# importZL/semantic_segmentation

Hardware: AMD Instinct MI355X
Metric: images/sec (fwd+bwd) U-Net 256x256 bs=32 per GPU (higher is better)
Workload: dtype f16; 1 GPU; unet.UNet(1,2) 256x256 fwd+bwd, CE+Dice loss, batch 32/GPU (BASELINE configs[1]); global_batch=32, parallelism=dp1, dice=per-rank

## Files before the change

### include/gsseg.h

```cpp
#ifndef GSSEG_H
#define GSSEG_H

#include <stdint.h>

#ifdef __cplusplus
extern "C" {
#endif

#define GS_ABI_VERSION 52

enum GsDtype { GS_F16 = 0, GS_BF16 = 1 };
enum GsStatus { GS_OK = 0, GS_EINVAL = -1, GS_ELAUNCH = -2, GS_EUNSUPPORTED = -3 };
enum GsAct { GS_ACT_NONE = 0, GS_ACT_RELU = 1, GS_ACT_LEAKY02 = 2, GS_ACT_TANH = 3 };

#define GS_MAX_TAPS 64

typedef struct GsConvGeom {
    int32_t N, IH, IW, Cin, in_pix_stride, in_coff;
    int32_t OHg, OWg, Cout;
    int32_t OH, OW, out_pix_stride, out_coff;
    int32_t isy, isx, osy, osx, ooy, oox;
    int32_t ntaps;
    int32_t tap_dy[GS_MAX_TAPS], tap_dx[GS_MAX_TAPS];
    int32_t tap_w[GS_MAX_TAPS];
// ... 85 lines not shown
                    int dtype, void* stream);

int gs_bn_bwd_tiles(int N, int H, int W);
int gs_bn_bwd_tiles_used(int N, int H, int W, int pooled);
int gs_bn_act_bwd_reduce(const void* y, const void* dz_a, int sa, int coff_a, const void* dzp,
                         const void* dz_b, int act_b, const uint8_t* keep_mask, float keep_scale,
                         const float* scale, const float* shift, const float* mean, const float* invstd, int act,
                         float* partials, int N, int H, int W, int C, int dtype, void* stream);
int gs_bn_bwd_coeffs(const float* partials, int ntiles, int C, double count, float gscale, float* dgamma,
                     float* dbeta, float* c1, float* c2, void* stream);
int gs_bn_act_bwd_apply(const void* y, const void* dz_a, int sa, int coff_a, const void* dzp,
                        const void* dz_b, int act_b, const uint8_t* keep_mask, float keep_scale,
                        const float* scale, const float* shift, const float* mean, const float* invstd,
                        const float* c1, const float* c2, int act, int bn, void* dy, int N, int H, int W, int C,
                        int dtype, void* stream);

int gs_maxpool3d_fwd(const void* z, int z_pix_stride, int z_coff, void* zp, int NB, int D, int H, int W, int C,
                     int dtype, void* stream);
int gs_maxpool3d_fwd_pair(const void* z_hi, const void* z_lo, int z_pix_stride, void* zp_hi, void* zp_lo, int zp_pix_stride,
                          int NB, int D, int H, int W, int C, int dtype, void* stream);
int gs_maxpool3d_fwd_pair_q8(const void* z_hi, const void* z_lo, int z_q8, int zq_coff, int z_pix_stride, void* zp_hi, void* zp_lo,
                             int zp_q8, int zp_pix_stride, int NB, int D, int H, int W, int C, int dtype, void* stream);
int gs_maxpool3d_bwd(const void* z, int z_pix_stride, int z_coff, const void* dzp, const void* dres,
                     int res_pix_stride, int res_coff, void* dz, int NB, int D, int H, int W, int C, int dtype,
                     void* stream);

int gs_maxpool2x2_fwd(const void* z, int z_pix_stride, int z_coff, void* zp, int N, int H, int W, int C, int dtype,
                      void* stream);
int gs_maxpool2x2_fwd_pair(const void* z_hi, const void* z_lo, int z_pix_stride, void* zp_hi, void* zp_lo, int zp_pix_stride, int N, int H,
                           int W, int C, int dtype, void* stream);
// ... 145 lines not shown
int gs_head1x1_bn_fwd_split(const void* y_hi, const void* y_lo, const float* scale, const float* shift, int act, const float* w,
                            const float* bias, float* logits, int N, int H, int W, int Cin, int Cout, int dtype, void* stream);
int gs_stem_fwd_bn_pair(const float* x, const float* w, const float* bn_scale, const float* bn_shift, int act, void* z_hi,
                        void* z_lo, int z_pix_stride, int N, int H, int W, int dtype, void* stream);
int gs_stem_bwd_onepass_strided(const float* x, const void* z, int z_pix_stride, const void* dz, int dz_stride, int dz_coff,
                                int act, float* s1_partials, float* ws, int N, int H, int W, int dtype, void* stream);

int gs_upconv2x2_wgrad_parts(int N, int IH, int IW, int Cin, int Cout);
int64_t gs_upconv2x2_wgrad_ws_floats(int N, int IH, int IW, int Cin, int Cout);
int gs_upconv2x2_wgrad_slabs(const void* x, const void* dy, float* ws, int N, int IH, int IW, int Cin, int x_pix_stride,
                             int x_coff, int Cout, int OH, int OW, int dy_pix_stride, int dy_coff, int ooy, int oox, int dtype,
                             void* stream);

int64_t gs_conv3x3_wgrad_ws_floats(int N, int H, int W, int Cin, int Cout);
int gs_conv3x3_wgrad_parts(int N, int H, int W, int Cin, int Cout);
int gs_conv3x3_wgrad_slabs(const void* x, const void* dy, float* ws, int N, int H, int W, int Cin, int in_pix_stride,
                           int in_coff, int Cout, int out_pix_stride, int out_coff, int dtype, void* stream);
int gs_wgrad_reduce_unpack(const float* ws, int nparts, float* grad, int A, int B, int taps, int transposed,
                           float gscale, void* stream);

int gs_conv3d_3x3x3_mtiles(int NB, int D, int H, int W, int Cout);
int gs_conv3d_3x3x3(const void* x, const void* w, void* y, const float* bias, float* bn_partials, int NB, int D, int H,
                    int W, int Cin, int in_pix_stride, int in_coff, int Cout, int out_pix_stride, int out_coff,
                    const int32_t* tap_dz, const int32_t* tap_dy, const int32_t* tap_dx, int act, int dtype, void* stream);
int gs_conv3d_3x3x3_wgrad(const void* x, const void* dy, float* dw, int NB, int D, int H, int W, int Cin,
                          int in_pix_stride, int in_coff, int Cout, int out_pix_stride, int out_coff, int dtype,
                          void* stream);
int64_t gs_conv3d_3x3x3_wgrad_ws_floats(int NB, int D, int H, int W, int Cin, int Cout);
int gs_conv3d_3x3x3_wgrad_parts(int NB, int D, int H, int W, int Cin, int Cout);
int gs_conv3d_3x3x3_wgrad_slabs(const void* x, const void* dy, float* ws, int NB, int D, int H, int W, int Cin,
// ... 29 lines not shown
```

### semantic_segmentation_amd/_lib.py

```python
from __future__ import annotations

import ctypes
import os
import subprocess
from ctypes import POINTER, c_char_p, c_double, c_float, c_int, c_int32, c_int64, c_void_p

_HERE = os.path.dirname(os.path.abspath(__file__))
LIB_PATH = os.environ.get("GSSEG_LIB", os.path.join(_HERE, "libgsseg_hip.so"))
CSRC = os.path.join(_HERE, "csrc")

GS_F16, GS_BF16 = 0, 1
ACT_NONE, ACT_RELU, ACT_LEAKY02, ACT_TANH = 0, 1, 2, 3
GS_MAX_TAPS = 64
ABI_VERSION = 52


class GsConvGeom(ctypes.Structure):
    _fields_ = [(n, c_int32) for n in (
        "N", "IH", "IW", "Cin", "in_pix_stride", "in_coff", "OHg", "OWg", "Cout", "OH", "OW",
        "out_pix_stride", "out_coff", "isy", "isx", "osy", "osx", "ooy", "oox", "ntaps")] + [
        ("tap_dy", c_int32 * GS_MAX_TAPS), ("tap_dx", c_int32 * GS_MAX_TAPS), ("tap_w", c_int32 * GS_MAX_TAPS)] + [
        (n, c_int32) for n in ("Dg", "Din", "Dout", "isz", "osz", "ooz")] + [("tap_dz", c_int32 * GS_MAX_TAPS)]


class GsPackDesc(ctypes.Structure):
    _fields_ = [("w", c_void_p), ("w_fwd", c_void_p), ("w_dgrad", c_void_p)] + [
        (n, c_int32) for n in ("Cout", "Cin", "taps", "transposed")]


# ... 32 lines not shown
    "gs_conv3d_3x3x3": (c_int, [_P, _P, _P, _F, _F] + [c_int] * 10 + [POINTER(c_int32)] * 3 + [c_int, c_int, c_void_p]),
    "gs_conv3d_3x3x3_wgrad_ws_floats": (c_int64, [c_int] * 6),
    "gs_conv3d_3x3x3_wgrad_parts": (c_int, [c_int] * 6),
    "gs_conv3d_3x3x3_wgrad_slabs": (c_int, [_P, _P, _F] + [c_int] * 11 + [c_void_p]),
    "gs_conv3d_3x3x3_wgrad": (c_int, [_P, _P, _F] + [c_int] * 11 + [c_void_p]),
    "gs_upsample2x_bilinear_fwd": (c_int, [_P, _P] + [c_int] * 13 + [c_void_p]),
    "gs_upsample2x_bilinear_bwd": (c_int, [_P, _P] + [c_int] * 13 + [c_void_p]),
    "gs_affine_warp": (c_int, [_F, _F, _F, c_int, c_int, c_int, c_int, c_float, c_void_p]),
    "gs_optim_chunk_elems": (c_int, []),
    "gs_optim_rmsprop": (c_int, [_P] * 7 + [c_int] + [c_float] * 6 + [c_void_p]),
    "gs_optim_adam": (c_int, [_P] * 7 + [c_int, _P] + [c_float] * 5 + [c_void_p]),
    "gs_conv3x3": (c_int, [_P, _P, _P, _F, _F] + [c_int] * 9 + [POINTER(c_int32), POINTER(c_int32), c_int, c_int, c_void_p]),
    "gs_conv3x3_wgrad": (c_int, [_P, _P, _F] + [c_int] * 10 + [c_void_p]),
    "gs_conv3x3_wgrad_ws_floats": (c_int64, [c_int] * 5),
    "gs_conv3x3_wgrad_parts": (c_int, [c_int] * 5),
    "gs_conv3x3_wgrad_slabs": (c_int, [_P, _P, _F] + [c_int] * 10 + [c_void_p]),
    "gs_wgrad_reduce_unpack": (c_int, [_F, c_int, _F, c_int, c_int, c_int, c_int, c_float, c_void_p]),
    "gs_conv_wgrad": (c_int, [POINTER(GsConvGeom), _P, _P, _F, c_int, c_void_p]),
    "gs_conv_wgrad_assign": (c_int, [POINTER(GsConvGeom), _P, _P, _F, c_int, c_void_p]),
    "gs_conv_wgrad_single_pass": (c_int, [POINTER(GsConvGeom)]),
    "gs_conv_wgrad_parts": (c_int, [POINTER(GsConvGeom)]),
    "gs_conv_wgrad_ws_floats": (c_int64, [POINTER(GsConvGeom)]),
    "gs_conv_wgrad_slabs": (c_int, [POINTER(GsConvGeom), _P, _P, _F, c_int, c_void_p]),
    "gs_conv_wgrad_slabs_batch": (c_int, [c_int, POINTER(POINTER(GsConvGeom)), _P, _P, _F, c_int, c_void_p]),
    "gs_conv_smallcin_mtiles": (c_int, [c_int, c_int, c_int]),
    "gs_conv_smallcin_fwd": (c_int, [_F, _F, _F, _P, _F] + [c_int] * 12 + [c_void_p]),
    "gs_conv_direct_wgrad_ws_floats": (c_int64, [c_int] * 6),
    "gs_conv_smallcin_wgrad": (c_int, [_F, _P, _F, _F] + [c_int] * 10 + [c_float, c_int, c_void_p]),
    "gs_conv_smallcin_dgrad": (c_int, [_P, _F, _F] + [c_int] * 10 + [c_float, c_int, c_void_p]),
    "gs_conv_smallcout_fwd": (c_int, [_P, _F, _F, _F] + [c_int] * 11 + [c_void_p]),
    "gs_conv_smallcout_bwd": (c_int, [_P, _F, _F, _P, _F, _F, _F] + [c_int] * 10 + [c_float, c_int, c_void_p]),
    "gs_bn_partials_floats": (c_int64, [c_int, c_int]),
    "gs_bn_finalize": (c_int, [_F, c_int, c_int, c_double, _F, _F, _F, _F, c_float, c_float, _F, _F, _F, _F, c_void_p]),
    "gs_bn_eval_coeffs": (c_int, [c_int, _F, _F, _F, _F, c_float, _F, _F, _F, _F, c_void_p]),
    "gs_bn_act_apply": (c_int, [_P, _F, _F, c_int, _P, c_int, c_int, _P, _P, c_float] + [c_int] * 5 + [c_void_p]),
    "gs_bn_bwd_tiles": (c_int, [c_int, c_int, c_int]),
    "gs_bn_bwd_tiles_used": (c_int, [c_int, c_int, c_int, c_int]),
    "gs_bn_act_bwd_reduce": (c_int, [_P, _P, c_int, c_int, _P, _P, c_int, _P, c_float, _F, _F, _F, _F, c_int, _F]
                             + [c_int] * 5 + [c_void_p]),
    "gs_bn_bwd_coeffs": (c_int, [_F, c_int, c_int, c_double, c_float, _F, _F, _F, _F, c_void_p]),
    "gs_bn_act_bwd_apply": (c_int, [_P, _P, c_int, c_int, _P, _P, c_int, _P, c_float, _F, _F, _F, _F, _F, _F, c_int,
                                    c_int, _P]
                            + [c_int] * 5 + [c_void_p]),
    "gs_maxpool3d_fwd": (c_int, [_P, c_int, c_int, _P] + [c_int] * 6 + [c_void_p]),
    "gs_maxpool2x2_fwd": (c_int, [_P, c_int, c_int, _P] + [c_int] * 5 + [c_void_p]),
    "gs_maxpool2x2_fwd_pair": (c_int, [_P, _P, c_int, _P, _P, c_int] + [c_int] * 5 + [c_void_p]),
    "gs_maxpool3d_bwd": (c_int, [_P, c_int, c_int, _P, _P, c_int, c_int, _P] + [c_int] * 6 + [c_void_p]),
    "gs_colsum": (c_int, [_P, c_int, c_int] + [c_int] * 8 + [c_float, _F, _F, c_int, c_void_p]),
    "gs_stem_bn_bwd_wgrad": (c_int, [_P, _P, c_int, c_int, _F, _F, _F, _F, _F, _F, _F, c_int, _F, _F, c_int, c_int, c_int,
                                     c_float, c_int, c_void_p]),
    "gs_stem_stats": (c_int, [_F, _F, _F, _F, c_int, c_int, c_int, c_void_p]),
    "gs_stem_bwd_onepass": (c_int, [_F, _P, _P, c_int, c_int, c_int, _F, _F, c_int, c_int, c_int, c_int, c_void_p]),
    "gs_stem_bwd_finalize": (c_int, [_F, _F, _F, _F, _F, _F, _F, c_int, c_float, _F, _F, _F, c_int, c_int, c_int, c_void_p]),
    "gs_stem_fwd_bn": (c_int, [_F, _F, _F, _F, c_int, _P, c_int, c_int, c_int, c_int, c_void_p]),
# ... 118 lines not shown
```

### semantic_segmentation_amd/csrc/bn.hip

```cpp
#include <stdlib.h>

#include "common.hpp"

namespace {

constexpr int RED_SLICES = 64;

__global__ __launch_bounds__(256) void reduce_partials_stage1(const float* __restrict__ part, int ntiles, int C,
                                                              int tiles_per_slice, double* __restrict__ out1) {
    __shared__ double red[2][8][32];
    const int cl = threadIdx.x & 31, tl = threadIdx.x >> 5;
    const int c = blockIdx.x * 32 + cl;
    const int t0 = blockIdx.y * tiles_per_slice, t1 = min(ntiles, t0 + tiles_per_slice);
    double s1 = 0.0, s2 = 0.0;
    if (c < C) {
        for (int tt = t0 + tl; tt < t1; tt += 8) {
            s1 += (double)part[((int64_t)tt * 2 + 0) * C + c];
            s2 += (double)part[((int64_t)tt * 2 + 1) * C + c];
        }
    }
    red[0][tl][cl] = s1;
    red[1][tl][cl] = s2;
    __syncthreads();
    if (tl == 0 && c < C) {
// ... 63 lines not shown
}

template <typename T>
__global__ __launch_bounds__(256) void bn_bwd_coeffs_kernel(const T* __restrict__ s, int nslices, int C, double count,
                                                            float gscale, float* dgamma, float* dbeta, float* c1, float* c2) {
    double s1, s2;
    sum_slices_32x8(s, nslices, C, s1, s2);
    const int c = blockIdx.x * 32 + (threadIdx.x & 31);
    if (c >= C || threadIdx.x >= 32) return;
    if (dbeta) dbeta[c] = (float)(s1 * gscale);
    if (dgamma) dgamma[c] = (float)(s2 * gscale);
    c1[c] = (float)(s1 / count);
    c2[c] = (float)(s2 / count);
}

static int bn_traversal() {
    static const int v = getenv("GSSEG_BN_REV") ? atoi(getenv("GSSEG_BN_REV")) : 3;
    return v;
}

struct ApplyArgs {
    const unsigned short* y;
    const float* scale;
    const float* shift;
    unsigned short* z;
    unsigned short* zp;
    const uint8_t* keep;
    float keep_scale;
    int act, N, H, W, C, zs, zc;
    int rev;
};

template <int DT, bool POOL, bool GENERIC>
// ... 77 lines not shown
    const unsigned short* dzb;
    const uint8_t* keep;
    float keep_scale;
    int act_b;
    const float *scale, *shift, *mean, *invstd, *c1, *c2;
    float* partials;
    unsigned short* dy;
    int sa, ca, act, bn, N, H, W, C;
    int tile_units;
    int rev;
    const float* head_dl;
    const float* head_w;
    int head_n;
};

template <int DT, bool POOL, bool APPLY, bool GENERIC, int HEAD = 0, bool EXTRA = true, bool RN = false>
__global__ __launch_bounds__(256) void bn_act_bwd_kernel(const BwdArgs a) {
    static_assert(!HEAD || (!POOL && !GENERIC), "the head source: plain pixels, slope-family activation");
    static_assert(!(RN && GENERIC), "the rounded slope product belongs to the slope family");
    auto mul_g = [&](float g, float d) __attribute__((always_inline)) { return RN ? mul_rn(g, d) : g * d; };
    constexpr int NH = HEAD ? HEAD : 1;
    constexpr int HEAD_CHUNK = 2048;
    __shared__ float hdl[HEAD ? NH * HEAD_CHUNK : 1];
    __shared__ float red[2][256 * 8 / 8][8];
    const float slope_a = a.act == GS_ACT_RELU ? 0.f : (a.act == GS_ACT_LEAKY02 ? 0.2f : 1.f);
    const float slope_b = a.act_b == GS_ACT_RELU ? 0.f : (a.act_b == GS_ACT_LEAKY02 ? 0.2f : 1.f);
    auto grad_a = [&](float v) __attribute__((always_inline)) { return GENERIC ? act_grad(v, a.act) : (v > 0.f ? 1.f : slope_a); };
    auto grad_b = [&](float v) __attribute__((always_inline)) { return GENERIC ? act_grad(v, a.act_b) : (v > 0.f ? 1.f : slope_b); };
    auto fwd_a = [&](float v) __attribute__((always_inline)) { return GENERIC ? act_fwd(v, a.act) : (v > 0.f ? v : v * slope_a); };
    const int nch = a.C >> 3;
    const int PH = POOL ? (a.H + 1) / 2 : a.H, PW = POOL ? (a.W + 1) / 2 : a.W;
    const int units = a.N * PH * PW;
    const int lanes_per_unit = nch < 256 ? nch : 256;
    const int unit_lanes = 256 / lanes_per_unit;
    const int chl = threadIdx.x % lanes_per_unit, ul = threadIdx.x / lanes_per_unit;
    const int tile = a.rev ? (int)(gridDim.x - 1 - blockIdx.x) : (int)blockIdx.x;
    const int u0 = tile * a.tile_units;
    int u1 = u0 + a.tile_units < units ? u0 + a.tile_units : units;
    if (ul >= unit_lanes) u1 = u0;
    constexpr int UNR = 4;

    for (int ch = chl; ch - chl < nch; ch += lanes_per_unit) {
        const bool ch_ok = ch < nch;
        const int c0 = ch_ok ? ch * 8 : 0;
        if (!ch_ok) u1 = u0;
        float sc[8], sh[8], mu[8], is[8], k1[8], k2[8];
#pragma unroll
        for (int i = 0; i < 8; ++i) {
            sc[i] = a.scale ? a.scale[c0 + i] : 1.f;
            sh[i] = a.shift ? a.shift[c0 + i] : 0.f;
            mu[i] = a.mean ? a.mean[c0 + i] : 0.f;
            is[i] = a.invstd ? a.invstd[c0 + i] : 1.f;
            k1[i] = (APPLY && a.c1) ? a.c1[c0 + i] : 0.f;
            k2[i] = (APPLY && a.c2) ? a.c2[c0 + i] : 0.f;
        }
// ... 361 lines not shown
    GS_CHECK_LAUNCH("gs_bn_act_apply");
    return GS_OK;
}

static int bwd_tile_units(int64_t units) {
    int64_t tu = cdiv64(units, 1024);
    if (tu < 64) tu = 64;
    return (int)tu;
}

extern "C" int gs_bn_bwd_tiles(int N, int H, int W) {
    const int64_t units = (int64_t)N * H * W;
    return (int)cdiv64(units, bwd_tile_units(units));
}

static int launch_bwd(const BwdArgs& a0, bool apply, int dtype, hipStream_t s, int* ntiles_out) {
    BwdArgs a = a0;
    a.rev = (bn_traversal() >> (apply ? 2 : 1)) & 1;
    const bool pool = a.dzp != nullptr;
    const int PH = pool ? (a.H + 1) / 2 : a.H, PW = pool ? (a.W + 1) / 2 : a.W;
    const int64_t units = (int64_t)a.N * PH * PW;
    const int ntiles_max = gs_bn_bwd_tiles(a.N, a.H, a.W);
    a.tile_units = (int)cdiv64(units, ntiles_max);
    if (a.tile_units < 1) a.tile_units = 1;
    const int ntiles = (int)cdiv64(units, a.tile_units);
    if (ntiles_out) *ntiles_out = ntiles;
    const bool generic = a.act == GS_ACT_TANH || (a.dzb && a.act_b == GS_ACT_TANH);
    const bool leaky = !generic && (a.act == GS_ACT_LEAKY02 || (a.dzb && a.act_b == GS_ACT_LEAKY02));
#define LAUNCH(DT, G, R)                                                                                \
    do {                                                                                                \
        if (pool) {                                                                                     \
            if (apply) bn_act_bwd_kernel<DT, true, true, G, 0, true, R><<<ntiles, 256, 0, s>>>(a);      \
            else bn_act_bwd_kernel<DT, true, false, G, 0, true, R><<<ntiles, 256, 0, s>>>(a);           \
        } else if (a.dzb != nullptr || a.keep != nullptr) {                                             \
            if (apply) bn_act_bwd_kernel<DT, false, true, G, 0, true, R><<<ntiles, 256, 0, s>>>(a);     \
            else bn_act_bwd_kernel<DT, false, false, G, 0, true, R><<<ntiles, 256, 0, s>>>(a);          \
        } else {                                                                                        \
            if (apply) bn_act_bwd_kernel<DT, false, true, G, 0, false, R><<<ntiles, 256, 0, s>>>(a);    \
            else bn_act_bwd_kernel<DT, false, false, G, 0, false, R><<<ntiles, 256, 0, s>>>(a);         \
        }                                                                                               \
    } while (0)
    if (a.head_dl != nullptr) {
#define LAUNCH_HEAD(DT, NC, R)                                                                          \
    do {                                                                                                \
        if (apply) bn_act_bwd_kernel<DT, false, true, false, NC, false, R><<<ntiles, 256, 0, s>>>(a);   \
        else bn_act_bwd_kernel<DT, false, false, false, NC, false, R><<<ntiles, 256, 0, s>>>(a);        \
    } while (0)
#define LAUNCH_HEAD_N(DT, R) do { if (a.head_n <= 2) LAUNCH_HEAD(DT, 2, R); else LAUNCH_HEAD(DT, 4, R); } while (0)
        if (dtype == GS_F16) { if (leaky) LAUNCH_HEAD_N(GS_F16, true); else LAUNCH_HEAD_N(GS_F16, false); }
        else { if (leaky) LAUNCH_HEAD_N(GS_BF16, true); else LAUNCH_HEAD_N(GS_BF16, false); }
#undef LAUNCH_HEAD_N
// ... 158 lines not shown
```

### semantic_segmentation_amd/csrc/wgrad3x3.hip

```cpp
#include <stdlib.h>

#include "common.hpp"

namespace {

struct W3Args {
    const unsigned short* x;
    const unsigned short* dy;
    float* dw;
    int N, H, W, Cin, in_stride, in_coff, Cout, out_stride, out_coff;
    int tiles_x, tiles_y, npatches, ncob, ncib, ksplit, pps;
    int D, dz;
    int64_t slab_stride;
};

constexpr int W3_LDR = 96;
constexpr int W3_BM = 128;

template <int DT, int TW>
__global__ __launch_bounds__(256, 2) void wgrad3x3_kernel(const W3Args a) {
    typedef typename Elem<DT>::V8 V8;
    constexpr int TH = W3_BM / TW;
    constexpr int HWD = TW + 2, HHT = TH + 2, HP = HWD * HHT;
    constexpr int DY_EL = W3_BM * W3_LDR, H_EL = HP * W3_LDR;
// ... 710 lines not shown
    const int64_t AB = (int64_t)A * B;
    if (!transposed && nparts <= rows_parts && AB >= 256 * 64 && AB < 2147483647LL / 64 && (taps == 9 || taps == 16 || taps == 4)) {
        const int nb = (int)cdiv64(AB, 256);
        hipStream_t s = (hipStream_t)stream;
        if (taps == 9) wgrad_reduce_rows_kernel<9><<<nb, 256, 0, s>>>(ws, nparts, n, grad, (int)AB, gscale);
        else if (taps == 16) wgrad_reduce_rows_kernel<16><<<nb, 256, 0, s>>>(ws, nparts, n, grad, (int)AB, gscale);
        else wgrad_reduce_rows_kernel<4><<<nb, 256, 0, s>>>(ws, nparts, n, grad, (int)AB, gscale);
        GS_CHECK_LAUNCH("gs_wgrad_reduce_unpack");
        return GS_OK;
    }
    wgrad_reduce_unpack_kernel<<<(int)cdiv64(n, 128), 256, 0, (hipStream_t)stream>>>(ws, nparts, n, grad, A, B, taps, transposed, gscale);
    GS_CHECK_LAUNCH("gs_wgrad_reduce_unpack");
    return GS_OK;
}

extern "C" int gs_conv3x3_wgrad_parts(int N, int H, int W, int Cin, int Cout) {
    return w3_ksplit(N, H, W, Cin, Cout, nullptr, nullptr, w3_use_dma(W));
}

extern "C" int64_t gs_conv3d_3x3x3_wgrad_ws_floats(int NB, int D, int H, int W, int Cin, int Cout) {
    if (NB <= 0 || D <= 0 || H <= 0 || W <= 0 || Cin <= 0 || Cout <= 0) return 0;
    return (int64_t)w3_ksplit(NB * D, H, W, Cin, Cout, nullptr, nullptr, w3_use_dma(W)) * 27 * Cout * Cin;
}

extern "C" int gs_conv3d_3x3x3_wgrad_parts(int NB, int D, int H, int W, int Cin, int Cout) {
    return w3_ksplit(NB * D, H, W, Cin, Cout, nullptr, nullptr, w3_use_dma(W));
}

extern "C" int gs_conv3d_3x3x3_wgrad_slabs(const void* x, const void* dy, float* ws, int NB, int D, int H, int W, int Cin,
                                           int in_pix_stride, int in_coff, int Cout, int out_pix_stride, int out_coff,
// ... 19 lines not shown
```

### semantic_segmentation_amd/ops.py

```python
from __future__ import annotations

import collections
import ctypes
import os
from typing import List, Optional, Sequence, Tuple

import torch

from . import _lib
from ._lib import ACT_NONE, GS_BF16, GS_F16, GsConvGeom

DTYPES = {"f16": (GS_F16, torch.float16), "bf16": (GS_BF16, torch.bfloat16)}


def dt_code(t: torch.Tensor) -> int:
    if t.dtype == torch.float16:
        return GS_F16
    if t.dtype == torch.bfloat16:
        return GS_BF16
    raise TypeError(f"expected a float16/bfloat16 tensor, got {t.dtype}")


def _p(t: Optional[torch.Tensor]):
    return None if t is None else t.data_ptr()
# ... 400 lines not shown


def upsample2x_bilinear_bwd(dy, dx, N, IH, IW, C, OH, OW, dy_stride=None, dy_coff=0, dx_stride=None, dx_coff=0,
                            ooy=0, oox=0):
    _dev(dy)
    if dy.dtype != dx.dtype:
        raise TypeError("upsample2x_bilinear_bwd: dy and dx must share one 16-bit dtype")
    _lib.call("gs_upsample2x_bilinear_bwd", _p(dy), _p(dx), N, IH, IW, C, C if dy_stride is None else dy_stride, dy_coff,
              OH, OW, C if dx_stride is None else dx_stride, dx_coff, ooy, oox, dt_code(dy), _stream())


def conv3x3_wgrad_parts(N, H, W, Cin, Cout) -> int:
    return int(_lib.load().gs_conv3x3_wgrad_parts(N, H, W, Cin, Cout))


def conv3x3_wgrad_ws_floats(N, H, W, Cin, Cout) -> int:
    return int(_lib.load().gs_conv3x3_wgrad_ws_floats(N, H, W, Cin, Cout))


def conv3x3_wgrad_det(x, dy, ws, grad, N, H, W, Cin, Cout, gscale, in_stride=None, in_coff=0, out_stride=None,
                      out_coff=0):
    _dev(x)
    _f32(ws, "ws"); _f32(grad, "grad")
    if x.dtype != dy.dtype:
        raise TypeError("conv3x3_wgrad_det: x and dy must share one 16-bit dtype")
    if ws.numel() < conv3x3_wgrad_ws_floats(N, H, W, Cin, Cout) or grad.numel() != 9 * Cout * Cin:
        raise ValueError("conv3x3_wgrad_det: workspace / gradient size")
    ev = TIMER.start() if TIMER is not None else None
    _lib.call("gs_conv3x3_wgrad_slabs", _p(x), _p(dy), _p(ws), N, H, W, Cin, Cin if in_stride is None else in_stride,
              in_coff, Cout, Cout if out_stride is None else out_stride, out_coff, dt_code(x), _stream())
# ... 269 lines not shown

def bn_act_apply(y, scale, shift, act, z, z_stride, z_coff, zp=None, keep_mask=None, keep_scale=1.0):
    N, H, W, C = y.shape
    if not y.is_contiguous():
        raise ValueError("bn_act_apply: y must be dense NHWC")
    _lib.call("gs_bn_act_apply", _p(y), _p(scale), _p(shift), act, _p(z), z_stride, z_coff, _p(zp), _p(keep_mask),
              float(keep_scale), N, H, W, C, dt_code(y), _stream())


def bn_bwd_tiles(N, H, W) -> int:
    return _lib.load().gs_bn_bwd_tiles(N, H, W)


def bn_bwd_tiles_used(N, H, W, pooled: bool) -> int:
    return _lib.load().gs_bn_bwd_tiles_used(N, H, W, int(pooled))


def bn_act_bwd_reduce(y, dz_a, sa, ca, dzp, scale, shift, mean, invstd, act, partials, dz_b=None, act_b=ACT_NONE,
                      keep_mask=None, keep_scale=1.0):
    N, H, W, C = y.shape
    _lib.call("gs_bn_act_bwd_reduce", _p(y), _p(dz_a), sa, ca, _p(dzp), _p(dz_b), act_b, _p(keep_mask),
              float(keep_scale), _p(scale), _p(shift), _p(mean), _p(invstd), act, _p(partials), N, H, W, C,
              dt_code(y), _stream())


def bn_bwd_coeffs(partials, ntiles, C, count, gscale, dgamma, dbeta, c1, c2):
    _lib.call("gs_bn_bwd_coeffs", _p(partials), ntiles, C, float(count), float(gscale), _p(dgamma), _p(dbeta),
              _p(c1), _p(c2), _stream())


# ... 664 lines not shown
```

### semantic_segmentation_amd/unet/unet_engine.py

```python
from __future__ import annotations

import functools
import math
import os
import warnings
from typing import Callable, Dict, List, Optional

import torch

from .. import ops
from .._lib import ACT_NONE, ACT_RELU
from ..engine_common import ParamIndex, _flush_nbt, bn_coeffs, compute_dtype, pack_key, pack_reuse_allowed

FOLD_BN_INFERENCE = os.environ.get("GSSEG_FOLD_BN", "1") != "0"
WGRAD_SIDE_STREAM = os.environ.get("GSSEG_WGRAD_STREAM", "0") != "0"
FUSED_STEM_BWD = os.environ.get("GSSEG_STEM_BWD_FUSED", "1") != "0"
FUSED_STEM_FWD = os.environ.get("GSSEG_STEM_FWD_FUSED", "1") != "0"
FUSED_HEAD_FWD = os.environ.get("GSSEG_HEAD_FWD_FUSED", "1") != "0"
FUSED_HEAD_BWD = os.environ.get("GSSEG_HEAD_BWD_FUSED", "1") != "0"
FUSED_UP_BIAS_GRAD = os.environ.get("GSSEG_UP_BIAS_FUSED", "1") != "0"


class _ConvRec:
    __slots__ = ("name", "wkey", "bnkey", "inp", "inp_is_image", "y", "coef", "geom", "cin", "cout", "h", "w",
                 "wd", "train_stats", "inp_stride", "z", "tap_sums", "wide")


class _UpRec:
    __slots__ = ("name", "zin", "cat", "geom_bwd", "geom_wg", "wd", "cin", "cout", "h", "w", "H2", "W2", "pt", "pl")

# ... 63 lines not shown

class UNetEngine(ParamIndex):

    def __init__(self, net, dtype: str = "f16", precise: bool = False):
        self.net = net
        self.dtype, self.tdt = compute_dtype(dtype)
        self.plan = resolve_plan(precise, self.dtype, bool(getattr(net, "bilinear", False)))
        self.precise = self.plan is not None
        self.auto = precise == "auto"
        self._warned_fallback = False
        self.dynamic_loss_scale = os.environ.get("GSSEG_DYNAMIC_LOSS_SCALE", "0") == "1"
        self._packs: Dict[str, tuple] = {}
        self.trust_versions = False
        self._side_streams: Dict[torch.device, torch.cuda.Stream] = {}
        self.grad_ready_hook: Optional[Callable[[str, torch.Tensor], None]] = None
        self.grad_alloc: Optional[Callable[[str, torch.Tensor], torch.Tensor]] = None
        self.after_backward: Optional[Callable[[], None]] = None
        self.grad_fetch: Optional[Callable[[str], torch.Tensor]] = None
        self.accumulate_grads = False

    def _side_stream(self, dev):
        st = self._side_streams.get(dev)
        if st is None:
            st = self._side_streams[dev] = torch.cuda.Stream(device=dev)
        return st

    def invalidate_packs(self):
        self._packs.clear()

    def _prepack(self, params: Dict[str, torch.Tensor], need_dgrad: bool, conv_fwd: bool = True):
# ... 611 lines not shown
            amax = dlogits.detach().abs().amax().float()
            k = torch.floor(-torch.log2(torch.clamp(amax * S, min=1e-30)))
            renorm = torch.exp2(torch.clamp(k, -60.0, 60.0))
            dlogits = dlogits * renorm
        grads: Dict[str, torch.Tensor] = {}

        def empty(*shape, dtype=tdt):
            return torch.empty(shape, dtype=dtype, device=dev)

        def emit(name, g):
            grads[name] = g
            if self.grad_ready_hook is not None:
                self.grad_ready_hook(name, g)

        main_stream = torch.cuda.current_stream(dev)
        side = self._side_stream(dev) if WGRAD_SIDE_STREAM else None
        deferred = []

        def flush_deferred(upto_all: bool):
            while deferred and (upto_all or len(deferred) > 1):
                name, g, ev = deferred.pop(0)
                main_stream.wait_event(ev)
                emit(name, g)

        def on_side(inputs, fn, name, g):
            if side is None:
                fn()
                emit(name, g)
                return
            ev = torch.cuda.Event()
            ev.record(main_stream)
            for t_ in inputs:
                t_.record_stream(side)
            with torch.cuda.stream(side):
                side.wait_event(ev)
                fn()
                if self.grad_ready_hook is not None:
                    done = torch.cuda.Event()
                    done.record(side)
                    deferred.append((name, g, done))
            if self.grad_ready_hook is None:
                grads[name] = g
            else:
                flush_deferred(False)
# ... 92 lines not shown
                        dgamma = galloc(rec.bnkey + ".weight", params[rec.bnkey + ".weight"])
                        dbeta = galloc(rec.bnkey + ".bias", params[rec.bnkey + ".bias"])
                        dw = galloc(rec.wkey, params[rec.wkey], zero=True)
                        ops.stem_bwd_finalize(sws, s1p, rec.tap_sums, wst, coef[0], coef[2], coef[3], rec.train_stats, inv_s,
                                              dw, dgamma, dbeta, N, h, w)
                        emit(rec.wkey, dw)
                        emit(rec.bnkey + ".weight", dgamma)
                        emit(rec.bnkey + ".bias", dbeta)
                        done = True
                if done:
                    return None
                y_re = empty(N, h, w, cout)
                ops.conv_smallcin_fwd(rec.inp, wst, None, y_re, None, 3, 1, 1)
                rec.y = y_re
            ntiles = ops.bn_bwd_tiles_used(N, h, w, pooled)
            if head is not None:
                ops.bn_act_bwd_reduce_head(rec.y, head[0], head[1], coef[0], coef[1], coef[2], coef[3], ACT_RELU, partials)
            else:
                ops.bn_act_bwd_reduce(rec.y, dz_a, sa, ca, dzp, coef[0], coef[1], coef[2], coef[3], ACT_RELU, partials)
            dgamma = galloc(rec.bnkey + ".weight", params[rec.bnkey + ".weight"])
            dbeta = galloc(rec.bnkey + ".bias", params[rec.bnkey + ".bias"])
            c12 = empty(2, cout, dtype=torch.float32)
            ops.bn_bwd_coeffs(partials, ntiles, cout, N * h * w, inv_s, dgamma, dbeta, c12[0], c12[1])
            if not rec.train_stats:
                c12.zero_()
            wparam = params[rec.wkey]
            dw_stem = None
            if (rec.inp_is_image and not need_dinp and not pooled and FUSED_STEM_BWD and cin == 1 and cout == 64
                    and rec.inp.is_contiguous()):
                dw_stem = galloc(rec.wkey, wparam, zero=True)
                if ops.stem_bn_bwd_wgrad(rec.y, dz_a, sa, ca, rec.inp, coef[0], coef[1], coef[2], coef[3], c12[0], c12[1],
                                         ACT_RELU, dw_stem, inv_s):
                    emit(rec.wkey, dw_stem)
                    emit(rec.bnkey + ".weight", dgamma)
                    emit(rec.bnkey + ".bias", dbeta)
                    return None
            dy = empty(N, h, w, cout)
            if head is not None:
                ops.bn_act_bwd_apply_head(rec.y, head[0], head[1], coef[0], coef[1], coef[2], coef[3], c12[0], c12[1], ACT_RELU, dy)
            else:
                ops.bn_act_bwd_apply(rec.y, dz_a, sa, ca, dzp, coef[0], coef[1], coef[2], coef[3], c12[0], c12[1],
                                     ACT_RELU, True, dy)
            dinp = None
            if rec.inp_is_image:
                dw = dw_stem if dw_stem is not None else galloc(rec.wkey, wparam, zero=True)
                ops.conv_smallcin_wgrad(rec.inp, dy, dw, 3, 1, 1, inv_s)
                if need_dinp:
                    dinp = torch.empty_like(rec.inp)
                    ops.conv_smallcin_dgrad(dy, wparam.detach().contiguous(), dinp, 3, 1, 1, inv_s)
            elif getattr(rec, "wide", 0):
                dwp = torch.empty((cout, cin, 3, 3), dtype=torch.float32, device=dev)
                ops.conv3x3_wgrad_det(rec.inp, dy, wg_ws, dwp, N, h, w, cin, cout, inv_s)
                dw = galloc(rec.wkey, wparam)
                dw.copy_(dwp[:, :rec.wide])
                wgrad_on_side = False
                if need_dinp:
                    dxp = empty(N, h, w, cin)
                    ops.conv3x3(dy, rec.wd, dxp, N, h, w, cout, cin, ops.TAPS3_DGRAD)
                    dfull = torch.empty((N, cin, h, w), dtype=torch.float32, device=dev)
                    ops.nhwc_to_nchw(dxp, dfull, gscale=inv_s)
                    dinp = dfull[:, :rec.wide].contiguous()
            else:
                dw = galloc(rec.wkey, wparam)
                wgrad_on_side = rec.name in det_recs
                if wgrad_on_side:
                    on_side((rec.inp, dy, wg_ws, dw),
                            lambda: ops.conv3x3_wgrad_det(rec.inp, dy, wg_ws, dw, N, h, w, cin, cout, inv_s, in_stride=rec.inp_stride),
                            rec.wkey, dw)
                else:
                    dwp = dw_take(wparam.numel())
                    if ops.USE_HALO_CONV and cin % 8 == 0 and cout % 8 == 0:
                        ops.conv3x3_wgrad(rec.inp, dy, dwp, N, h, w, cin, cout, in_stride=rec.inp_stride)
                    else:
                        ops.conv_wgrad(rec.geom, rec.inp, dy, dwp)
                    ops.unpack_wgrad(dwp, dw, cout, cin, 9, False, inv_s)
                if need_dinp:
                    dinp = empty(N, h, w, cin)
                    if ops.USE_HALO_CONV and rec.inp_stride is None and rec.train_stats and stream_conv(N, h, w, cout, cin):
                        gd = ops.geom_conv_dgrad_s1(N, h, w, cin, cout, 3, 1)
                        if colsum is not None:
                            ops.conv_igemm(gd, dy, rec.wd, dinp, None, partials)
                            ops.bn_partials_colsum(partials, ops.conv_igemm_mtiles(gd), cin, colsum[0], colsum[1], inv_s, colsum[2])
                        else:
                            ops.conv_igemm(gd, dy, rec.wd, dinp)
                    elif ops.USE_HALO_CONV and colsum is not None:
                        ops.conv3x3(dy, rec.wd, dinp, N, h, w, cout, cin, ops.TAPS3_DGRAD, bn_partials=partials)
                        ops.bn_partials_colsum(partials, ops.conv3x3_stat_rows(N, h, w, cout, cin), cin, colsum[0], colsum[1], inv_s, colsum[2])
                    elif ops.USE_HALO_CONV:
                        ops.conv3x3(dy, rec.wd, dinp, N, h, w, cout, cin, ops.TAPS3_DGRAD)
                    else:
                        ops.conv_igemm(ops.geom_conv_dgrad_s1(N, h, w, cin, cout, 3, 1), dy, rec.wd, dinp)
            if rec.inp_is_image or not wgrad_on_side:
                emit(rec.wkey, dw)
            emit(rec.bnkey + ".weight", dgamma)
            emit(rec.bnkey + ".bias", dbeta)
            return dinp

        dcats = [None] * 4
        for j in range(4, 0, -1):
            lvl = 4 - j
            prefix = f"up{j}"
            cout_t = C[lvl]
            r3, r0 = recs[prefix + ".conv.3"], recs[prefix + ".conv.0"]
            dmid = conv_stage_bwd(r3, dz, r3.cout, 0, None, True, head=head_src if j == 4 else None)
            u = ups[prefix]
            db_fused = None
# ... 4 lines not shown
                                  colsum=None if db_fused is None else (cout_t, cout_t, db_fused))
            dcats[lvl] = dcat
            if u.geom_bwd is None:
                dz = empty(N, u.h, u.w, u.cin)
                ops.upsample2x_bilinear_bwd(dcat, dz, N, u.h, u.w, u.cin, u.H2, u.W2, dy_stride=2 * cout_t,
                                            dy_coff=cout_t, ooy=u.pt, oox=u.pl)
                continue
            wkey = prefix + ".up.weight"
            wparam = params[wkey]
            if db_fused is not None:
                db = db_fused
            else:
                db = galloc(prefix + ".up.bias", params[prefix + ".up.bias"])
                ops.colsum(dcat, 2 * cout_t, cout_t, N, u.H2, u.W2, u.pt, u.pl, 2 * u.h, 2 * u.w, cout_t, inv_s, col_ws, db)
            dw = galloc(wkey, wparam)
            on_side((dcat, u.zin, wg_ws, dw),
                    lambda u=u, dcat=dcat, dw=dw: ops.upconv2x2_wgrad_det(
                        u.geom_wg if u.geom_wg is not None else u.geom_bwd, u.zin, dcat, wg_ws, dw, N, u.h, u.w, u.cin, u.cout,
                        u.H2, u.W2, u.zin.shape[3], 2 * u.cout, u.cout, u.pt, u.pl, inv_s),
                    wkey, dw)
            dz = empty(N, u.h, u.w, u.cin)
            ops.upconv2x2_dgrad(u.geom_bwd, dcat, u.wd, dz, N, u.h, u.w, u.cin, u.cout, u.H2, u.W2, 2 * cout_t, cout_t, u.pt, u.pl)
            emit(prefix + ".up.bias", db)

        dx = None
        dpool = None
        for i in range(4, -1, -1):
            prefix = "inc" if i == 0 else f"down{i}.maxpool_conv.1"
            if i == 4:
                dmid = conv_stage_bwd(recs[prefix + ".3"], dz, C[i], 0, None, True)
            else:
                dmid = conv_stage_bwd(recs[prefix + ".3"], dcats[i], 2 * C[i], 0, dpool, True)
            r0 = recs[prefix + ".0"]
            dinp = conv_stage_bwd(r0, dmid, C[i], 0, None, (i > 0) or need_dx)
            if i > 0:
                dpool = dinp
            else:
# ... 52 lines not shown
```

Before: 2157 images/sec.

## Enable wgrad side stream by default with slim BN-backward kernel during overlap

Turns the weight-gradient side stream on by default, except under graph capture. Conv3x3 and upconv wgrad launches move after their dgrad so the two overlap. While a side-stream wgrad is in flight, the BN backward reduce and apply kernels switch to a slim variant with smaller unroll and higher occupancy bounds, to share the GPU better. The side stream is joined before DMA-family wgrads and before wide-channel wgrads, which adds stream-sync overhead and contention risk.

```diff
diff --git a/include/gsseg.h b/include/gsseg.h
--- a/include/gsseg.h
+++ b/include/gsseg.h
@@ -7,7 +7,7 @@
 extern "C" {
 #endif
 
-#define GS_ABI_VERSION 52
+#define GS_ABI_VERSION 53
 
 enum GsDtype { GS_F16 = 0, GS_BF16 = 1 };
 enum GsStatus { GS_OK = 0, GS_EINVAL = -1, GS_ELAUNCH = -2, GS_EUNSUPPORTED = -3 };
@@ -123,6 +123,8 @@
                         const float* scale, const float* shift, const float* mean, const float* invstd,
                         const float* c1, const float* c2, int act, int bn, void* dy, int N, int H, int W, int C,
                         int dtype, void* stream);
+int gs_bn_bwd_set_form(int form);
+int gs_bn_set_traversal(int mask);
 
 int gs_maxpool3d_fwd(const void* z, int z_pix_stride, int z_coff, void* zp, int NB, int D, int H, int W, int C,
                      int dtype, void* stream);
@@ -298,6 +300,7 @@
 
 int64_t gs_conv3x3_wgrad_ws_floats(int N, int H, int W, int Cin, int Cout);
 int gs_conv3x3_wgrad_parts(int N, int H, int W, int Cin, int Cout);
+int gs_conv3x3_wgrad_family(int W, int Cout);
 int gs_conv3x3_wgrad_slabs(const void* x, const void* dy, float* ws, int N, int H, int W, int Cin, int in_pix_stride,
                            int in_coff, int Cout, int out_pix_stride, int out_coff, int dtype, void* stream);
 int gs_wgrad_reduce_unpack(const float* ws, int nparts, float* grad, int A, int B, int taps, int transposed,
diff --git a/semantic_segmentation_amd/_lib.py b/semantic_segmentation_amd/_lib.py
--- a/semantic_segmentation_amd/_lib.py
+++ b/semantic_segmentation_amd/_lib.py
@@ -12,7 +12,7 @@
 GS_F16, GS_BF16 = 0, 1
 ACT_NONE, ACT_RELU, ACT_LEAKY02, ACT_TANH = 0, 1, 2, 3
 GS_MAX_TAPS = 64
-ABI_VERSION = 52
+ABI_VERSION = 53
 
 
 class GsConvGeom(ctypes.Structure):
@@ -75,6 +75,7 @@
     "gs_conv3x3_wgrad": (c_int, [_P, _P, _F] + [c_int] * 10 + [c_void_p]),
     "gs_conv3x3_wgrad_ws_floats": (c_int64, [c_int] * 5),
     "gs_conv3x3_wgrad_parts": (c_int, [c_int] * 5),
+    "gs_conv3x3_wgrad_family": (c_int, [c_int] * 2),
     "gs_conv3x3_wgrad_slabs": (c_int, [_P, _P, _F] + [c_int] * 10 + [c_void_p]),
     "gs_wgrad_reduce_unpack": (c_int, [_F, c_int, _F, c_int, c_int, c_int, c_int, c_float, c_void_p]),
     "gs_conv_wgrad": (c_int, [POINTER(GsConvGeom), _P, _P, _F, c_int, c_void_p]),
@@ -99,6 +100,8 @@
     "gs_bn_bwd_tiles_used": (c_int, [c_int, c_int, c_int, c_int]),
     "gs_bn_act_bwd_reduce": (c_int, [_P, _P, c_int, c_int, _P, _P, c_int, _P, c_float, _F, _F, _F, _F, c_int, _F]
                              + [c_int] * 5 + [c_void_p]),
+    "gs_bn_bwd_set_form": (c_int, [c_int]),
+    "gs_bn_set_traversal": (c_int, [c_int]),
     "gs_bn_bwd_coeffs": (c_int, [_F, c_int, c_int, c_double, c_float, _F, _F, _F, _F, c_void_p]),
     "gs_bn_act_bwd_apply": (c_int, [_P, _P, c_int, c_int, _P, _P, c_int, _P, c_float, _F, _F, _F, _F, _F, _F, c_int,
                                     c_int, _P]
diff --git a/semantic_segmentation_amd/csrc/bn.hip b/semantic_segmentation_amd/csrc/bn.hip
--- a/semantic_segmentation_amd/csrc/bn.hip
+++ b/semantic_segmentation_amd/csrc/bn.hip
@@ -101,9 +101,15 @@
     c2[c] = (float)(s2 / count);
 }
 
+static int g_traversal = -1;
 static int bn_traversal() {
     static const int v = getenv("GSSEG_BN_REV") ? atoi(getenv("GSSEG_BN_REV")) : 3;
-    return v;
+    return g_traversal >= 0 ? g_traversal : v;
+}
+extern "C" int gs_bn_set_traversal(int mask) {
+    GS_CHECK_ARG(mask >= -1 && mask <= 7, "gs_bn_set_traversal: mask must be -1 (GSSEG_BN_REV / default) or 0..7");
+    g_traversal = mask;
+    return GS_OK;
 }
 
 struct ApplyArgs {
@@ -211,10 +217,11 @@
     int head_n;
 };
 
-template <int DT, bool POOL, bool APPLY, bool GENERIC, int HEAD = 0, bool EXTRA = true, bool RN = false>
-__global__ __launch_bounds__(256) void bn_act_bwd_kernel(const BwdArgs a) {
+template <int DT, bool POOL, bool APPLY, bool GENERIC, int HEAD = 0, bool EXTRA = true, bool RN = false, bool SLIM = false>
+__global__ __launch_bounds__(256, SLIM ? 5 : 1) void bn_act_bwd_kernel(const BwdArgs a) {
     static_assert(!HEAD || (!POOL && !GENERIC), "the head source: plain pixels, slope-family activation");
     static_assert(!(RN && GENERIC), "the rounded slope product belongs to the slope family");
+    static_assert(!SLIM || (!POOL && !GENERIC && !HEAD && !EXTRA && !RN), "the slim form: the plain U-Net launch only");
     auto mul_g = [&](float g, float d) __attribute__((always_inline)) { return RN ? mul_rn(g, d) : g * d; };
     constexpr int NH = HEAD ? HEAD : 1;
     constexpr int HEAD_CHUNK = 2048;
@@ -235,7 +242,7 @@
     const int u0 = tile * a.tile_units;
     int u1 = u0 + a.tile_units < units ? u0 + a.tile_units : units;
     if (ul >= unit_lanes) u1 = u0;
-    constexpr int UNR = 4;
+    constexpr int UNR = SLIM ? 2 : 4;
 
     for (int ch = chl; ch - chl < nch; ch += lanes_per_unit) {
         const bool ch_ok = ch < nch;
@@ -627,6 +634,13 @@
     return (int)cdiv64(units, bwd_tile_units(units));
 }
 
+static int g_bwd_form = 0;
+extern "C" int gs_bn_bwd_set_form(int form) {
+    GS_CHECK_ARG(form == 0 || form == 1, "gs_bn_bwd_set_form: form must be 0 (normal) or 1 (slim)");
+    g_bwd_form = form;
+    return GS_OK;
+}
+
 static int launch_bwd(const BwdArgs& a0, bool apply, int dtype, hipStream_t s, int* ntiles_out) {
     BwdArgs a = a0;
     a.rev = (bn_traversal() >> (apply ? 2 : 1)) & 1;
@@ -648,6 +662,10 @@
         } else if (a.dzb != nullptr || a.keep != nullptr) {                                             \
             if (apply) bn_act_bwd_kernel<DT, false, true, G, 0, true, R><<<ntiles, 256, 0, s>>>(a);     \
             else bn_act_bwd_kernel<DT, false, false, G, 0, true, R><<<ntiles, 256, 0, s>>>(a);          \
+        } else if (g_bwd_form == 1 && !(G) && !(R)) {    \
+            constexpr bool S = !(G) && !(R);                                                            \
+            if (apply) bn_act_bwd_kernel<DT, false, true, G, 0, false, R, S><<<ntiles, 256, 0, s>>>(a); \
+            else bn_act_bwd_kernel<DT, false, false, G, 0, false, R, S><<<ntiles, 256, 0, s>>>(a);      \
         } else {                                                                                        \
             if (apply) bn_act_bwd_kernel<DT, false, true, G, 0, false, R><<<ntiles, 256, 0, s>>>(a);    \
             else bn_act_bwd_kernel<DT, false, false, G, 0, false, R><<<ntiles, 256, 0, s>>>(a);         \
diff --git a/semantic_segmentation_amd/csrc/wgrad3x3.hip b/semantic_segmentation_amd/csrc/wgrad3x3.hip
--- a/semantic_segmentation_amd/csrc/wgrad3x3.hip
+++ b/semantic_segmentation_amd/csrc/wgrad3x3.hip
@@ -748,6 +748,10 @@
     return GS_OK;
 }
 
+extern "C" int gs_conv3x3_wgrad_family(int W, int Cout) {
+    return w3_use_co128(W, Cout) ? 2 : (w3_use_dma(W) ? 1 : 0);
+}
+
 extern "C" int gs_conv3x3_wgrad_parts(int N, int H, int W, int Cin, int Cout) {
     return w3_ksplit(N, H, W, Cin, Cout, nullptr, nullptr, w3_use_dma(W));
 }
diff --git a/semantic_segmentation_amd/ops.py b/semantic_segmentation_amd/ops.py
--- a/semantic_segmentation_amd/ops.py
+++ b/semantic_segmentation_amd/ops.py
@@ -1,6 +1,7 @@
 from __future__ import annotations
 
 import collections
+import contextlib
 import ctypes
 import os
 from typing import List, Optional, Sequence, Tuple
@@ -438,6 +439,10 @@
     return int(_lib.load().gs_conv3x3_wgrad_parts(N, H, W, Cin, Cout))
 
 
+def conv3x3_wgrad_family(W, Cout) -> int:
+    return int(_lib.load().gs_conv3x3_wgrad_family(W, Cout))
+
+
 def conv3x3_wgrad_ws_floats(N, H, W, Cin, Cout) -> int:
     return int(_lib.load().gs_conv3x3_wgrad_ws_floats(N, H, W, Cin, Cout))
 
@@ -737,6 +742,29 @@
 
 def bn_bwd_tiles_used(N, H, W, pooled: bool) -> int:
     return _lib.load().gs_bn_bwd_tiles_used(N, H, W, int(pooled))
+
+
+BN_BWD_NORMAL, BN_BWD_SLIM = 0, 1
+
+
+def bn_bwd_set_form(form: int = BN_BWD_NORMAL) -> None:
+    _lib.call("gs_bn_bwd_set_form", int(form))
+
+
+def bn_set_traversal(mask: int = -1) -> None:
+    _lib.call("gs_bn_set_traversal", int(mask))
+
+
+@contextlib.contextmanager
+def bn_bwd_form(form: int):
+    if form == BN_BWD_NORMAL:
+        yield
+        return
+    bn_bwd_set_form(form)
+    try:
+        yield
+    finally:
+        bn_bwd_set_form(BN_BWD_NORMAL)
 
 
 def bn_act_bwd_reduce(y, dz_a, sa, ca, dzp, scale, shift, mean, invstd, act, partials, dz_b=None, act_b=ACT_NONE,
diff --git a/semantic_segmentation_amd/unet/unet_engine.py b/semantic_segmentation_amd/unet/unet_engine.py
--- a/semantic_segmentation_amd/unet/unet_engine.py
+++ b/semantic_segmentation_amd/unet/unet_engine.py
@@ -13,7 +13,7 @@
 from ..engine_common import ParamIndex, _flush_nbt, bn_coeffs, compute_dtype, pack_key, pack_reuse_allowed
 
 FOLD_BN_INFERENCE = os.environ.get("GSSEG_FOLD_BN", "1") != "0"
-WGRAD_SIDE_STREAM = os.environ.get("GSSEG_WGRAD_STREAM", "0") != "0"
+WGRAD_SIDE_STREAM = os.environ.get("GSSEG_WGRAD_STREAM", "1") != "0"
 FUSED_STEM_BWD = os.environ.get("GSSEG_STEM_BWD_FUSED", "1") != "0"
 FUSED_STEM_FWD = os.environ.get("GSSEG_STEM_FWD_FUSED", "1") != "0"
 FUSED_HEAD_FWD = os.environ.get("GSSEG_HEAD_FWD_FUSED", "1") != "0"
@@ -107,6 +107,7 @@
         self.trust_versions = False
         self._side_streams: Dict[torch.device, torch.cuda.Stream] = {}
         self.grad_ready_hook: Optional[Callable[[str, torch.Tensor], None]] = None
+        self.last_backward_streams = 0
         self.grad_alloc: Optional[Callable[[str, torch.Tensor], torch.Tensor]] = None
         self.after_backward: Optional[Callable[[], None]] = None
         self.grad_fetch: Optional[Callable[[str], torch.Tensor]] = None
@@ -748,8 +749,12 @@
                 self.grad_ready_hook(name, g)
 
         main_stream = torch.cuda.current_stream(dev)
-        side = self._side_stream(dev) if WGRAD_SIDE_STREAM else None
+        two_streams = WGRAD_SIDE_STREAM and not torch.cuda.is_current_stream_capturing()
+        self.last_backward_streams = 2 if two_streams else 1
+        side = self._side_stream(dev) if two_streams else None
         deferred = []
+        side_busy = [False]
+        slim_bn = [False]
 
         def flush_deferred(upto_all: bool):
             while deferred and (upto_all or len(deferred) > 1):
@@ -757,11 +762,19 @@
                 main_stream.wait_event(ev)
                 emit(name, g)
 
-        def on_side(inputs, fn, name, g):
-            if side is None:
+        def join_side():
+            if side is not None and side_busy[0]:
+                flush_deferred(True)
+                main_stream.wait_stream(side)
+                side_busy[0] = slim_bn[0] = False
+
+        def on_side(inputs, fn, name, g, beside=True, leaves_96=False):
+            if side is None or not beside:
+                join_side()
                 fn()
                 emit(name, g)
                 return
+            side_busy[0], slim_bn[0] = True, leaves_96
             ev = torch.cuda.Event()
             ev.record(main_stream)
             for t_ in inputs:
@@ -884,10 +897,12 @@
                 ops.conv_smallcin_fwd(rec.inp, wst, None, y_re, None, 3, 1, 1)
                 rec.y = y_re
             ntiles = ops.bn_bwd_tiles_used(N, h, w, pooled)
+            slim = slim_bn[0] and not pooled and head is None
             if head is not None:
                 ops.bn_act_bwd_reduce_head(rec.y, head[0], head[1], coef[0], coef[1], coef[2], coef[3], ACT_RELU, partials)
             else:
-                ops.bn_act_bwd_reduce(rec.y, dz_a, sa, ca, dzp, coef[0], coef[1], coef[2], coef[3], ACT_RELU, partials)
+                with ops.bn_bwd_form(ops.BN_BWD_SLIM if slim else ops.BN_BWD_NORMAL):
+                    ops.bn_act_bwd_reduce(rec.y, dz_a, sa, ca, dzp, coef[0], coef[1], coef[2], coef[3], ACT_RELU, partials)
             dgamma = galloc(rec.bnkey + ".weight", params[rec.bnkey + ".weight"])
             dbeta = galloc(rec.bnkey + ".bias", params[rec.bnkey + ".bias"])
             c12 = empty(2, cout, dtype=torch.float32)
@@ -909,8 +924,9 @@
             if head is not None:
                 ops.bn_act_bwd_apply_head(rec.y, head[0], head[1], coef[0], coef[1], coef[2], coef[3], c12[0], c12[1], ACT_RELU, dy)
             else:
-                ops.bn_act_bwd_apply(rec.y, dz_a, sa, ca, dzp, coef[0], coef[1], coef[2], coef[3], c12[0], c12[1],
-                                     ACT_RELU, True, dy)
+                with ops.bn_bwd_form(ops.BN_BWD_SLIM if slim else ops.BN_BWD_NORMAL):
+                    ops.bn_act_bwd_apply(rec.y, dz_a, sa, ca, dzp, coef[0], coef[1], coef[2], coef[3], c12[0], c12[1],
+                                         ACT_RELU, True, dy)
             dinp = None
             if rec.inp_is_image:
                 dw = dw_stem if dw_stem is not None else galloc(rec.wkey, wparam, zero=True)
@@ -920,6 +936,7 @@
                     ops.conv_smallcin_dgrad(dy, wparam.detach().contiguous(), dinp, 3, 1, 1, inv_s)
             elif getattr(rec, "wide", 0):
                 dwp = torch.empty((cout, cin, 3, 3), dtype=torch.float32, device=dev)
+                join_side()
                 ops.conv3x3_wgrad_det(rec.inp, dy, wg_ws, dwp, N, h, w, cin, cout, inv_s)
                 dw = galloc(rec.wkey, wparam)
                 dw.copy_(dwp[:, :rec.wide])
@@ -933,11 +950,7 @@
             else:
                 dw = galloc(rec.wkey, wparam)
                 wgrad_on_side = rec.name in det_recs
-                if wgrad_on_side:
-                    on_side((rec.inp, dy, wg_ws, dw),
-                            lambda: ops.conv3x3_wgrad_det(rec.inp, dy, wg_ws, dw, N, h, w, cin, cout, inv_s, in_stride=rec.inp_stride),
-                            rec.wkey, dw)
-                else:
+                if not wgrad_on_side:
                     dwp = dw_take(wparam.numel())
                     if ops.USE_HALO_CONV and cin % 8 == 0 and cout % 8 == 0:
                         ops.conv3x3_wgrad(rec.inp, dy, dwp, N, h, w, cin, cout, in_stride=rec.inp_stride)
@@ -960,6 +973,11 @@
                         ops.conv3x3(dy, rec.wd, dinp, N, h, w, cout, cin, ops.TAPS3_DGRAD)
                     else:
                         ops.conv_igemm(ops.geom_conv_dgrad_s1(N, h, w, cin, cout, 3, 1), dy, rec.wd, dinp)
+                if wgrad_on_side:
+                    fam = ops.conv3x3_wgrad_family(w, cout)
+                    on_side((rec.inp, dy, wg_ws, dw),
+                            lambda: ops.conv3x3_wgrad_det(rec.inp, dy, wg_ws, dw, N, h, w, cin, cout, inv_s, in_stride=rec.inp_stride),
+                            rec.wkey, dw, beside=fam != 1, leaves_96=True)
             if rec.inp_is_image or not wgrad_on_side:
                 emit(rec.wkey, dw)
             emit(rec.bnkey + ".weight", dgamma)
@@ -994,13 +1012,13 @@
                 db = galloc(prefix + ".up.bias", params[prefix + ".up.bias"])
                 ops.colsum(dcat, 2 * cout_t, cout_t, N, u.H2, u.W2, u.pt, u.pl, 2 * u.h, 2 * u.w, cout_t, inv_s, col_ws, db)
             dw = galloc(wkey, wparam)
+            dz = empty(N, u.h, u.w, u.cin)
+            ops.upconv2x2_dgrad(u.geom_bwd, dcat, u.wd, dz, N, u.h, u.w, u.cin, u.cout, u.H2, u.W2, 2 * cout_t, cout_t, u.pt, u.pl)
             on_side((dcat, u.zin, wg_ws, dw),
                     lambda u=u, dcat=dcat, dw=dw: ops.upconv2x2_wgrad_det(
                         u.geom_wg if u.geom_wg is not None else u.geom_bwd, u.zin, dcat, wg_ws, dw, N, u.h, u.w, u.cin, u.cout,
                         u.H2, u.W2, u.zin.shape[3], 2 * u.cout, u.cout, u.pt, u.pl, inv_s),
                     wkey, dw)
-            dz = empty(N, u.h, u.w, u.cin)
-            ops.upconv2x2_dgrad(u.geom_bwd, dcat, u.wd, dz, N, u.h, u.w, u.cin, u.cout, u.H2, u.W2, 2 * cout_t, cout_t, u.pt, u.pl)
             emit(prefix + ".up.bias", db)
 
         dx = None
```

Result: faster. 2201 images/sec (median of 6 runs) (+2.0%).
